# M2219/pyOrbSLAM

Measured on AMD Instinct MI355X. Metric: stereo pairs/s (ORB extract L+R + stereo match), KITTI 1241x376, 1/2/4/8 GPU, higher is better.
Workload: dtype u8; 1 GPU; kitti1241x376_synth_2000f_512pairs; width=1241, height=376, nfeatures=2000, nlevels=8, iniThFAST=20, minThFAST=7, parallelism=512 pairs per GPU on 1 GPU(s) (independent ranks, no data-path collective), handles_per_gpu=4, lanes_per_handle=1

## Files before the change

### pyorbslam_amd/csrc/orbfe_kernels.hip

```cpp
#include <hip/hip_runtime.h>

#include <algorithm>
#include <mutex>
#include <vector>

#include "orbfe_common.h"
#include <type_traits>

#include "orbfe_kernels.h"

namespace orbfe {

constexpr int kBriefSlots = 384;
#define BRIEF_POINT(x, y) x, y,
#define BRIEF_BIT(s0, s1)
constexpr float kBriefSlotXY[2 * kBriefSlots] = {
#include "brief_distinct.inc"
};
#undef BRIEF_POINT
#undef BRIEF_BIT
#define BRIEF_SLOT(s) s,
constexpr int kBriefSlotOrder[kBriefSlots] = {
#include "brief_slot_order.inc"
};
// ... 37 lines not shown
    const uint32_t hi = __builtin_amdgcn_readfirstlane((uint32_t)(a >> 32));
    return __builtin_amdgcn_make_buffer_rsrc((void*)(uintptr_t)(((uint64_t)hi << 32) | lo), 0,
                                             __builtin_amdgcn_readfirstlane(nbytes), 0x00020000);
}

__device__ __forceinline__ __amdgpu_buffer_rsrc_t aligned_rsrc(const void* p, uint32_t nbytes, uint32_t* bias) {
    const uint64_t a = (uint64_t)(uintptr_t)p;
    const uint32_t lo = __builtin_amdgcn_readfirstlane((uint32_t)a);
    const uint32_t hi = __builtin_amdgcn_readfirstlane((uint32_t)(a >> 32));
    *bias = lo & 3u;
    const uint32_t nb = __builtin_amdgcn_readfirstlane(nbytes);
    return __builtin_amdgcn_make_buffer_rsrc((void*)(uintptr_t)(((uint64_t)hi << 32) | (lo & ~3u)), 0, nb + (lo & 3u),
                                             0x00020000);
}

__device__ __forceinline__ void wave_sum2(int& a, int& b) {
    a += __builtin_amdgcn_update_dpp(0, a, 0xB1, 0xF, 0xF, false);
    b += __builtin_amdgcn_update_dpp(0, b, 0xB1, 0xF, 0xF, false);
    a += __builtin_amdgcn_update_dpp(0, a, 0x4E, 0xF, 0xF, false);
    b += __builtin_amdgcn_update_dpp(0, b, 0x4E, 0xF, 0xF, false);
    a += __builtin_amdgcn_update_dpp(0, a, 0x124, 0xF, 0xF, false);
    b += __builtin_amdgcn_update_dpp(0, b, 0x124, 0xF, 0xF, false);
    a += __builtin_amdgcn_update_dpp(0, a, 0x128, 0xF, 0xF, false);
    b += __builtin_amdgcn_update_dpp(0, b, 0x128, 0xF, 0xF, false);
    a = __builtin_amdgcn_readlane(a, 0) + __builtin_amdgcn_readlane(a, 16) + __builtin_amdgcn_readlane(a, 32) +
        __builtin_amdgcn_readlane(a, 48);
    b = __builtin_amdgcn_readlane(b, 0) + __builtin_amdgcn_readlane(b, 16) + __builtin_amdgcn_readlane(b, 32) +
        __builtin_amdgcn_readlane(b, 48);
}

__device__ __forceinline__ int wave_sum(int v) {
    v += __builtin_amdgcn_update_dpp(0, v, 0xB1, 0xF, 0xF, false);
    v += __builtin_amdgcn_update_dpp(0, v, 0x4E, 0xF, 0xF, false);
    v += __builtin_amdgcn_update_dpp(0, v, 0x124, 0xF, 0xF, false);
    v += __builtin_amdgcn_update_dpp(0, v, 0x128, 0xF, 0xF, false);
    return __builtin_amdgcn_readlane(v, 0) + __builtin_amdgcn_readlane(v, 16) + __builtin_amdgcn_readlane(v, 32) +
           __builtin_amdgcn_readlane(v, 48);
}

__device__ __forceinline__ int reflect101(int p, int n) {
    p = p < 0 ? -p : p;
    return p >= n ? 2 * n - 2 - p : p;
}

__device__ __forceinline__ int reflect101_iter(int p, int n) {
    if (n == 1) return 0;
    const int per = 2 * n - 2;
    p = (p < 0 ? -p : p) % per;
    return p >= n ? per - p : p;
}

__device__ __forceinline__ uint32_t resize_tail(uint32_t t, int area) {
    if (!area) return (t + (1u << 21)) >> 22;
    const uint32_t q = t >> 22, r = t & 0x3FFFFFu;
    return q + (r > 0x200000u || (r == 0x200000u && (q & 1u)));
}

__device__ __forceinline__ const uint8_t* level_ptr(const Geo& g, int l, const uint8_t* in, int64_t in_pitch,
                                                    const uint8_t* ws, int img, int* stride) {
    if (l == 0) {
        *stride = g.W;
        return in + (int64_t)img * in_pitch;
    }
    *stride = g.lv[l].pitch;
    return ws + (int64_t)img * g.ws_bytes + g.lv[l].ws_off;
}

__device__ __forceinline__ CellGeo load_cell(const CellGeo* __restrict__ cells, int c) {
    static_assert(sizeof(CellGeo) == 20, "CellGeo layout: 5 dwords");
    const uint32_t* p = (const uint32_t*)(cells + c);
    const uint32_t w0 = p[0], w1 = p[1], w2 = p[2], w3 = p[3], w4 = p[4];
    CellGeo cg;
    cg.level = (int16_t)(w0 & 0xFFFFu);
    cg.kw = (int16_t)(w0 >> 16);
    cg.x0 = (int16_t)(w1 & 0xFFFFu);
    cg.y0 = (int16_t)(w1 >> 16);
    cg.x1 = (int16_t)(w2 & 0xFFFFu);
    cg.y1 = (int16_t)(w2 >> 16);
    cg.slot_off = (int)w3;
    cg.slot_cap = (int)w4;
    return cg;
}

struct KeyDiv {
    uint32_t w, mag, sh;
};
__device__ __forceinline__ KeyDiv key_div(const LevelGeo& L) {
    return KeyDiv{(uint32_t)__builtin_amdgcn_readfirstlane(L.w), (uint32_t)__builtin_amdgcn_readfirstlane((int)L.kmag),
                  (uint32_t)__builtin_amdgcn_readfirstlane(L.ksh)};
}
__device__ __forceinline__ void key_xy(uint32_t k, KeyDiv kd, int& x, int& y) {
    const uint32_t xy = k & 0xFFFFFFu;
    const uint32_t q = __umulhi(xy, kd.mag) >> kd.sh;
    y = (int)q;
    x = (int)(xy - __umul24(q, kd.w));
}

__device__ __forceinline__ void xcd_block(int& bx, int& by) {
    const int nb = gridDim.x * gridDim.y, hw = blockIdx.y * gridDim.x + blockIdx.x, per = nb >> 3;
    const int lb = hw < 8 * per ? (hw & 7) * per + (hw >> 3) : hw;
    by = __builtin_amdgcn_readfirstlane(lb / (int)gridDim.x);
    bx = __builtin_amdgcn_readfirstlane(lb - by * (int)gridDim.x);
}

__device__ int block_excl_scan(int* a, int n, int* tmp) {
    const int t = threadIdx.x;
    const int per = (n + 255) >> 8;
    const int b = t < 256 ? min(t * per, n) : n, e = min(b + per, n);
    int s = 0;
    for (int i = b; i < e; ++i) s += a[i];
    if (t < 256) tmp[t] = s;
    __syncthreads();
    if (t < 64) {
        const int v0 = tmp[4 * t], v1 = tmp[4 * t + 1], v2 = tmp[4 * t + 2], v3 = tmp[4 * t + 3];
        const int tot = v0 + v1 + v2 + v3;
        int inc = tot;
#pragma unroll
        for (int o = 1; o < 64; o <<= 1) {
            const int y = __shfl_up(inc, o, 64);
            if (t >= o) inc += y;
        }
        const int ex = inc - tot;
        tmp[4 * t] = ex;
        tmp[4 * t + 1] = ex + v0;
        tmp[4 * t + 2] = ex + v0 + v1;
        tmp[4 * t + 3] = ex + v0 + v1 + v2;
        if (t == 63) tmp[256] = inc;
    }
    __syncthreads();
    int run = t < 256 ? tmp[t] : 0;
    for (int i = b; i < e; ++i) {
        const int v = a[i];
        a[i] = run;
        run += v;
    }
    const int total = tmp[256];
    __syncthreads();
    return total;
}

__device__ int block_sum(int v, int* red) {
    v = wave_sum(v);
    const int w = threadIdx.x >> 6, nw = blockDim.x >> 6;
    if ((threadIdx.x & 63) == 0) red[w] = v;
    __syncthreads();
    int s = 0;
    for (int i = 0; i < nw; ++i) s += red[i];
    __syncthreads();
    return s;
}

typedef unsigned short us2 __attribute__((ext_vector_type(2)));

__device__ __forceinline__ uint32_t resize_tap3(uint32_t A3, uint32_t aa) {
    typedef __attribute__((address_space(3))) const uint32_t lds_c32;
    const uint32_t o = A3 & 3u;
    lds_c32* w = (lds_c32*)(uintptr_t)(A3 - o);
    const uint32_t x = __builtin_amdgcn_alignbyte(w[1], w[0], o);
    return __builtin_amdgcn_udot2(__builtin_bit_cast(us2, __builtin_amdgcn_perm(x, x, 0x0c010c00u)),
                                  __builtin_bit_cast(us2, aa), 0u, false);
}
constexpr int kRsSlots = 16;

template <bool MULTI>
__global__ __launch_bounds__(512) void k_resize_rows(Geo g, int l, const uint8_t* __restrict__ in, int64_t in_pitch,
                                                     uint8_t* __restrict__ ws, const ResizeX* __restrict__ xt,
                                                     const ResizeY* __restrict__ yt, int wg, int remw, int wgl,
                                                     int* __restrict__ zero_word) {
    extern __shared__ __attribute__((aligned(16))) unsigned char rs_lds[];
    typedef __attribute__((address_space(3))) uint32_t lds_w32;
    typedef __attribute__((address_space(1))) const uint32_t glb_u32;
    lds_w32* s_src = (lds_w32*)(uintptr_t)(__attribute__((address_space(3))) unsigned char*)rs_lds;
    const LevelGeo& L = g.lv[l];
    const LevelGeo& P = g.lv[l - 1];
    int bx, img;
    xcd_block(bx, img);
    const int t = threadIdx.x, nthr = blockDim.x;
    if (zero_word && blockIdx.x == 0 && blockIdx.y == 0 && t == 0) *zero_word = 0;
    const int rows = L.rs_rows;
    const int dy0 = bx * rows, nrow = min(rows, L.h - dy0);
    const int ngrp = (L.w + 3) >> 2;
    int sstride;
    const uint8_t* src = level_ptr(g, l - 1, in, in_pitch, ws, img, &sstride);
    const ResizeY* yb = yt + L.ytab_off + dy0;
    const int ys_lo = yb[0].sy0, ys_hi = yb[nrow - 1].sy1;
    const uintptr_t a0 = (uintptr_t)(src + (int64_t)ys_lo * sstride);
    const int sh0 = (int)(a0 & 3);
    glb_u32* gsrc = (glb_u32*)(a0 - sh0);
    const int ndw = ((ys_hi - ys_lo) * sstride + P.w + sh0 + 3) >> 2;
    typedef __attribute__((address_space(3))) const uint32_t lds_u32;
    const uint32_t src_lds = (uint32_t)(uintptr_t)s_src;
    const int wv = t >> 6, fullw = (nthr >> 6) - remw, nset = fullw / wgl;
    const bool remwave = wv >= fullw;
    const int set = __builtin_amdgcn_readfirstlane(remwave ? 0 : wv / wgl);
    const int rem = ngrp - wg * 64, lane = t & 63;
    const int rstep = remwave ? 64 / rem : nset;
    const int row0 = remwave ? lane / rem : set;
    int ch = remwave ? wg : wv - set * wgl;
    const int ch_step = remwave ? 1 : wgl, ch_end = remwave ? wg + 1 : wg;
    int grp = 0;
    bool own = false;
    uint4 e{}, aa{};
    int sx0 = 0;
    uint32_t d3 = 0;
    auto chunk = [&](int c) {
        grp = remwave ? wg * 64 + lane % rem : c * 64 + lane;
        own = remwave ? lane < rstep * rem : grp < ngrp;
        if (own) {
            const uint4* xg = (const uint4*)(xt + L.xtab_off);
            const uint4 q0 = xg[2 * grp], q1 = xg[2 * grp + 1];
            sx0 = (int)q0.x;
            d3 = q1.z - q0.x;
            auto sel = [&](uint32_t sx) { const uint32_t r = sx - q0.x; return r | ((r + 1) << 16) | 0x0c000c00u; };
            e = uint4{sel(q0.x), sel(q0.z), sel(q1.x), sel(q1.z)};
            aa = uint4{q0.y, q0.w, q1.y, q1.w};
        }
    };
    chunk(ch);
    if (t < 256) {
        const __amdgpu_buffer_rsrc_t rsrc = bounded_rsrc((const void*)(uintptr_t)gsrc, (uint32_t)(4 * ndw));
        for (int base = 0; base < ndw; base += 256 * kRsSlots) {
            const int left = ndw - base;
            uint32_t v[kRsSlots];
#pragma unroll
            for (int k = 0; k < kRsSlots; ++k) {
                v[k] = 0u;
                if (t < left - 256 * k)
                    v[k] = __builtin_amdgcn_raw_buffer_load_b32(rsrc, (uint32_t)(4 * t), (uint32_t)(4 * (base + 256 * k)), 0);
            }
            lds_w32* sp = s_src + base + t;
#pragma unroll
            for (int k = 0; k < kRsSlots; ++k)
                if (t < left - 256 * k) sp[256 * k] = v[k];
        }
    }
    __syncthreads();
    uint8_t* dst = ws + (int64_t)img * g.ws_bytes + L.ws_off + (int64_t)dy0 * L.pitch;
    const __amdgpu_buffer_rsrc_t rd = uniform_rsrc(dst);
    for (;;) {
        if (!own) return;
        const int dx = 4 * grp;
        const bool tail = dx + 3 >= L.xvec;
        const uint32_t lsrc = src_lds + (uint32_t)sh0 + (uint32_t)sx0;
        int psy = -1;
        auto row = [&](int rr, uint32_t (&h0)[4], uint32_t (&h1)[4], bool reuse) {
            const ResizeY y = yb[rr];
            const uint32_t r0 = (uint32_t)((y.sy0 - ys_lo) * sstride), r1 = (uint32_t)((y.sy1 - ys_lo) * sstride);
            const uint32_t B0 = (uint32_t)y.b0 << 12, B1 = (uint32_t)y.b1 << 12;
            auto taps = [&](uint32_t roff, uint32_t (&h)[4]) {
                const uint32_t A = lsrc + roff, o = A & 3u;
                lds_u32* w = (lds_u32*)(uintptr_t)(A - o);
                const uint32_t w0 = w[0], w1 = w[1], w2 = w[2];
                const uint32_t d0 = __builtin_amdgcn_alignbyte(w1, w0, o), d1 = __builtin_amdgcn_alignbyte(w2, w1, o);
                h[0] = __builtin_amdgcn_udot2(__builtin_bit_cast(us2, __builtin_amdgcn_perm(d1, d0, e.x)),
                                              __builtin_bit_cast(us2, aa.x), 0u, false);
                h[1] = __builtin_amdgcn_udot2(__builtin_bit_cast(us2, __builtin_amdgcn_perm(d1, d0, e.y)),
                                              __builtin_bit_cast(us2, aa.y), 0u, false);
                h[2] = __builtin_amdgcn_udot2(__builtin_bit_cast(us2, __builtin_amdgcn_perm(d1, d0, e.z)),
                                              __builtin_bit_cast(us2, aa.z), 0u, false);
                h[3] = L.wide ? resize_tap3(A + d3, aa.w)
                              : __builtin_amdgcn_udot2(__builtin_bit_cast(us2, __builtin_amdgcn_perm(d1, d0, e.w)),
                                                       __builtin_bit_cast(us2, aa.w), 0u, false);
            };
            if (!(reuse && y.sy0 == psy)) taps(r0, h0);
            taps(r1, h1);
            if (reuse) psy = y.sy1;
            uint32_t v[4];
#pragma unroll
            for (int k = 0; k < 4; ++k) v[k] = (__umulhi(h0[k] & ~15u, B0) + __umulhi(h1[k] & ~15u, B1) + 2) >> 2;
            if (tail) {
#pragma unroll
                for (int k = 0; k < 4; ++k)
                    if (dx + k >= L.xvec) v[k] = resize_tail(h0[k] * (B0 >> 12) + h1[k] * (B1 >> 12), L.area);
            }
            __builtin_amdgcn_raw_buffer_store_b32(v[0] | (v[1] << 8) | (v[2] << 16) | (v[3] << 24), rd, (uint32_t)dx,
                                                  (uint32_t)(rr * L.pitch), 0);
        };
        uint32_t ha[4] = {0u, 0u, 0u, 0u}, hb[4] = {0u, 0u, 0u, 0u};
        if (!remwave) {
            const int per = (nrow + nset - 1) / nset, rend = min(set * per + per, nrow);
            psy = -1;
            int rr = set * per;
            for (; rr + 1 < rend; rr += 2) {
                row(rr, ha, hb, true);
                row(rr + 1, hb, ha, true);
            }
            if (rr < rend) row(rr, ha, hb, true);
        } else {
            for (int rr = row0; rr < nrow; rr += rstep) row(rr, ha, hb, false);
        }
        if (!MULTI) return;
        ch += ch_step;
        if (ch >= ch_end) return;
        chunk(ch);
    }
}

constexpr int kCasNT = 1024;
__global__ __launch_bounds__(kCasNT) void k_resize_cascade(Geo g, const uint8_t* __restrict__ in, int64_t in_pitch,
                                                        uint8_t* __restrict__ ws, const ResizeX* __restrict__ xt,
                                                        const ResizeY* __restrict__ yt, const int16_t* __restrict__ tab,
                                                        int offB, int offX, int* __restrict__ zero_word,
                                                        long long* __restrict__ prof) {
    extern __shared__ __attribute__((aligned(16))) unsigned char rs_lds[];
    typedef __attribute__((address_space(3))) const uint32_t lds_u32;
    typedef __attribute__((address_space(3))) uint32_t lds_w32;
    const int strip = blockIdx.x, img = blockIdx.y, t = threadIdx.x, lane = t & 63;
    const int wv = __builtin_amdgcn_readfirstlane(t >> 6), nwv = blockDim.x >> 6;
    if (zero_word && strip == 0 && img == 0 && t == 0) *zero_word = 0;
    long long* pm = prof ? prof + ((int64_t)img * gridDim.x + strip) * 32 : nullptr;
    auto mark = [&](int id) {
        if (pm && t == 0) pm[id] = (long long)wall_clock64();
    };
    mark(0);
    const int L = g.nlevels;
    const int16_t* st = tab + (int64_t)strip * L * 4;
    const uint32_t baseA = (uint32_t)(uintptr_t)(lds_u32*)rs_lds;
    const uint32_t baseB = baseA + (uint32_t)offB;
    typedef unsigned int v4u __attribute__((ext_vector_type(4)));
    typedef __attribute__((address_space(3))) v4u lds_u4;
    typedef __attribute__((address_space(3))) int lds_i32;
    typedef __attribute__((address_space(1))) const v4u glb_u4;
    auto u4 = [](v4u v) { return uint4{v.x, v.y, v.z, v.w}; };
    typedef __attribute__((address_space(1))) const uint32_t glb_u32;
    auto s_xa_of = [&](int par) { return (lds_u4*)(uintptr_t)(baseA + (uint32_t)offX + (uint32_t)(par * 32 * g.rs_ngrp)); };
    auto s_sx_of = [&](int par) {
        return (lds_i32*)(uintptr_t)(baseA + (uint32_t)offX + (uint32_t)(64 * g.rs_ngrp + par * 4 * g.rs_ngrp));
    };
    constexpr int kPre = 1024 / kCasNT;
    uint4 pq0[kPre], pq1[kPre];
    auto prefetch = [&](int l) {
        if (l >= g.nlevels) return;
        glb_u4* xg = (glb_u4*)(xt + g.lv[l].xtab_off);
        const int ng = (g.lv[l].w + 3) >> 2;
#pragma unroll
        for (int k = 0; k < kPre; ++k) {
            const int gi = t + kCasNT * k;
            if (gi < ng) {
                pq0[k] = u4(xg[2 * gi]);
                pq1[k] = u4(xg[2 * gi + 1]);
            }
        }
    };
    auto commit = [&](int l) {
        lds_u4* sxa = s_xa_of(l & 1);
        lds_i32* ssx = s_sx_of(l & 1);
        const int ng = (g.lv[l].w + 3) >> 2;
#pragma unroll
        for (int k = 0; k < kPre; ++k) {
            const int gi = t + kCasNT * k;
            if (gi < ng) {
                const uint4 q0 = pq0[k], q1 = pq1[k];
                auto sel = [&](uint32_t sx) { const uint32_t r = sx - q0.x; return r | ((r + 1) << 16) | 0x0c000c00u; };
                sxa[2 * gi] = v4u{sel(q0.x), sel(q0.z), sel(q1.x), sel(q1.z)};
                sxa[2 * gi + 1] = v4u{q0.y, q0.w, q1.y, q1.w};
                ssx[gi] = (int)(q0.x | ((q1.z - q0.x) << 24));
            }
        }
    };
    prefetch(1);
    uint32_t src_base = baseA, src_sh;
    int src_row0, src_stride;
    {
        const LevelGeo& L1 = g.lv[1];
        const ResizeY* yb = yt + L1.ytab_off;
        const int c0 = st[4], c1 = st[5];
        const int ys_lo = yb[c0].sy0, ys_hi = yb[c1 - 1].sy1;
        const uintptr_t a0 = (uintptr_t)(in + (int64_t)img * in_pitch + (int64_t)ys_lo * g.W);
        src_sh = (uint32_t)(a0 & 3);
        glb_u32* gsrc = (glb_u32*)(a0 - src_sh);
        const int ndw = ((ys_hi - ys_lo) * g.W + g.W + (int)src_sh + 3) >> 2;
        lds_w32* s_src = (lds_w32*)(uintptr_t)baseA;
        for (int base = 0; base < ndw; base += kCasNT * kRsSlots / 2) {
            uint32_t v[kRsSlots / 2];
#pragma unroll
            for (int k = 0; k < kRsSlots / 2; ++k) {
                const int i = base + t + kCasNT * k;
                v[k] = i < ndw ? gsrc[i] : 0u;
            }
#pragma unroll
            for (int k = 0; k < kRsSlots / 2; ++k) {
                const int i = base + t + kCasNT * k;
                if (i < ndw) s_src[i] = v[k];
            }
        }
        src_row0 = ys_lo;
        src_stride = g.W;
    }
    mark(1);
    for (int l = 1; l < L; ++l) {
        const LevelGeo& Lv = g.lv[l];
        const int c0 = st[4 * l], c1 = st[4 * l + 1], o0 = st[4 * l + 2], o1 = st[4 * l + 3];
        const int ngrp = (Lv.w + 3) >> 2, nch = (ngrp + 63) >> 6;
        commit(l);
        prefetch(l + 1);
        const lds_u4* s_xa = s_xa_of(l & 1);
        const lds_i32* s_sx0 = s_sx_of(l & 1);
        const ResizeY* yb = yt + Lv.ytab_off;
        const uint32_t dst_base = (l & 1) ? baseB : baseA;
        __syncthreads();
        mark(2 + l);
        uint8_t* gdst = ws + (int64_t)img * g.ws_bytes + Lv.ws_off;
        const int pitch = Lv.pitch;
        const int lv_wide = __builtin_amdgcn_readfirstlane(Lv.wide), lv_xvec = __builtin_amdgcn_readfirstlane(Lv.xvec),
                  lv_area = __builtin_amdgcn_readfirstlane(Lv.area);
        for (int r = c0 + wv; r < c1; r += nwv) {
            const ResizeY y = yb[r];
            const uint32_t r0 = (uint32_t)((y.sy0 - src_row0) * src_stride), r1 = (uint32_t)((y.sy1 - src_row0) * src_stride);
            const uint32_t B0 = (uint32_t)y.b0 << 12, B1 = (uint32_t)y.b1 << 12;
            const bool own = r >= o0 && r < o1;
            const uint32_t lrow = dst_base + (uint32_t)((r - c0) * pitch);
            uint8_t* grow = gdst + (int64_t)r * pitch;
            for (int ch = 0; ch < nch; ++ch) {
                const int grp = ch * 64 + lane;
                if (grp < ngrp) {
                    const uint4 e = u4(s_xa[2 * grp]), aa = u4(s_xa[2 * grp + 1]);
                    const int sxp = s_sx0[grp];
                    const uint32_t d3 = (uint32_t)sxp >> 24;
                    const uint32_t lsrc = src_base + src_sh + (uint32_t)(sxp & 0xFFFFFF);
                    auto taps = [&](uint32_t roff, uint32_t (&h)[4]) {
                        const uint32_t A = lsrc + roff, o = A & 3u;
                        lds_u32* w = (lds_u32*)(uintptr_t)(A - o);
                        const uint32_t w0 = w[0], w1 = w[1], w2 = w[2];
                        const uint32_t d0 = __builtin_amdgcn_alignbyte(w1, w0, o), d1 = __builtin_amdgcn_alignbyte(w2, w1, o);
                        h[0] = __builtin_amdgcn_udot2(__builtin_bit_cast(us2, __builtin_amdgcn_perm(d1, d0, e.x)),
                                                      __builtin_bit_cast(us2, aa.x), 0u, false);
                        h[1] = __builtin_amdgcn_udot2(__builtin_bit_cast(us2, __builtin_amdgcn_perm(d1, d0, e.y)),
                                                      __builtin_bit_cast(us2, aa.y), 0u, false);
                        h[2] = __builtin_amdgcn_udot2(__builtin_bit_cast(us2, __builtin_amdgcn_perm(d1, d0, e.z)),
                                                      __builtin_bit_cast(us2, aa.z), 0u, false);
                        h[3] = lv_wide ? resize_tap3(A + d3, aa.w)
                                       : __builtin_amdgcn_udot2(__builtin_bit_cast(us2, __builtin_amdgcn_perm(d1, d0, e.w)),
                                                                __builtin_bit_cast(us2, aa.w), 0u, false);
                    };
                    uint32_t h0[4], h1[4];
                    taps(r0, h0);
                    taps(r1, h1);
                    const int dx = 4 * grp;
                    uint32_t v[4];
#pragma unroll
                    for (int k = 0; k < 4; ++k) v[k] = (__umulhi(h0[k] & ~15u, B0) + __umulhi(h1[k] & ~15u, B1) + 2) >> 2;
                    if (dx + 3 >= lv_xvec) {
#pragma unroll
// ... 2725 lines not shown
                if (rtk) mR &= mR - 1;
                else mL &= mL - 1;
                if (slot == k) {
                    own = ownk;
                    rt = rtk;
                    ok = okk;
                }
            }
            const int orow = __shfl(wrow, own, 64), ocl = __shfl(c0l, own, 64), ocr = __shfl(c0r, own, 64);
            const int oct = __shfl(kl.octave, own, 64);
            if (ok && jb < (rt ? 21 : 11)) {
                const int w = s_w[oct], h = s_h[oct], pw = w + 2 * kEdge;
                const int stride = oct == 0 ? g.W : s_pitch[oct];
                int r, c;
                sheared_pos(w, orow, rt ? ocr : ocl, r, c);
                c += jb;
                if (c >= pw) {
                    c -= pw;
                    ++r;
                }
                const uint8_t* base = oct == 0 ? (rt ? lvl0R : lvl0L) : (rt ? wsR : wsL) + s_wsoff[oct];
                const uint16_t e = (uint16_t)(base[(int64_t)reflect101(r - kEdge, h) * stride + reflect101(c - kEdge, w)] + 512u);
                const int gq = (int)(threadIdx.x >> 6) * 4 + (own >> 4), gs = own & 15;
                if (rt) {
                    ((uint16_t*)&sE[gq][gs][0])[jb] = e;
                    if (jb >= 1) ((uint16_t*)&sO[gq][gs][0])[jb - 1] = e;
                } else {
                    ((uint16_t*)&sP[gq][gs][0])[jb] = e;
                }
            }
        }
    }
    __builtin_amdgcn_fence(__ATOMIC_RELEASE, "wavefront");
    __builtin_amdgcn_wave_barrier();
    __builtin_amdgcn_fence(__ATOMIC_ACQUIRE, "wavefront");
    if (do_sad && sl < 11) {
        const int s = sl;
        const int lc = (int)((sP[kq][5][2] >> 16) & 0xFFFFu);
        const uint32_t rw = sE[kq][5][(s + 5) >> 1];
        const int rc = (int)((s & 1) ? (rw & 0xFFFFu) : (rw >> 16));
        const uint32_t d = (uint32_t)(rc - lc) & 0xFFFFu;
        const uint32_t dd = d | (d << 16);
        const int b0 = s >> 1;
        uint32_t acc = 0;
#pragma unroll
        for (int r = 0; r < 11; ++r) {
            const uint32_t* bp = (s & 1) ? &sO[kq][r][b0] : &sE[kq][r][b0];
#pragma unroll
            for (int k = 0; k < 6; ++k) {
                const uint32_t a = __builtin_bit_cast(uint32_t, __builtin_bit_cast(us2, sP[kq][r][k]) +
                                                                    __builtin_bit_cast(us2, dd));
                const uint32_t b = bp[k];
                acc = k < 5 ? __builtin_amdgcn_sad_u16(a, b, acc) : __builtin_amdgcn_sad_u16(a & 0xFFFFu, b & 0xFFFFu, acc);
            }
        }
        sad[kq][s] = (int)acc;
    }
    __builtin_amdgcn_fence(__ATOMIC_RELEASE, "wavefront");
    __builtin_amdgcn_wave_barrier();
    __builtin_amdgcn_fence(__ATOMIC_ACQUIRE, "wavefront");
    if (do_sad && sl == 0) {
        int bi = 0, bd = sad[kq][0];
        for (int s = 1; s < 11; ++s)
            if (sad[kq][s] < bd) {
                bd = sad[kq][s];
                bi = s;
            }
        if (bi != 0 && bi != 10) {
            const int d1 = sad[kq][bi - 1], d2 = sad[kq][bi], d3 = sad[kq][bi + 1];
            const float deltaR = __fdiv_rn((float)(d1 - d3), (float)(2 * (d1 + d3 - 2 * d2)));
            if (!(deltaR < -1.f || deltaR > 1.f)) {
                const float bestuR = __fmul_rn(s_sc[kl.octave], __fadd_rn((float)(scaleduR0 + bi - 5), deltaR));
                const float disparity = __fsub_rn(kl.x, bestuR);
                if (0.f <= disparity && disparity < A.maxD) {
                    if (disparity <= 0.f) {
                        status = 2;
                        uR = (float)((double)kl.x - 0.01);
                        depth = (float)(A.bf / 0.01);
                    } else {
                        status = 1;
                        uR = bestuR;
                        depth = __fdiv_rn(A.bf32, disparity);
                    }
                }
            }
        }
    }
    if (active && sl == 0) {
        const int64_t o = pr * A.out_stride + iL;
        A.u_right[o] = status ? uR : -1.f;
        A.depth[o] = status ? depth : -1.f;
        A.status[o] = (int8_t)status;
        A.match_r[o] = status ? bidx : -1;
    }
}

__global__ __launch_bounds__(256) void k_hamming_matrix(const uint8_t* __restrict__ a, int na, const uint8_t* __restrict__ b,
                                                        int nb, int* __restrict__ out) {
    const int j = blockIdx.x * blockDim.x + threadIdx.x, i = blockIdx.y;
    if (j >= nb) return;
    const uint4* A4 = (const uint4*)(a + (int64_t)i * 32);
    const uint4* B4 = (const uint4*)(b + (int64_t)j * 32);
    const uint4 a0 = A4[0], a1 = A4[1], b0 = B4[0], b1 = B4[1];
    out[(int64_t)i * nb + j] = __popc(a0.x ^ b0.x) + __popc(a0.y ^ b0.y) + __popc(a0.z ^ b0.z) + __popc(a0.w ^ b0.w) +
                               __popc(a1.x ^ b1.x) + __popc(a1.y ^ b1.y) + __popc(a1.z ^ b1.z) + __popc(a1.w ^ b1.w);
}

__global__ __launch_bounds__(256) void k_hamming_search(const uint8_t* __restrict__ q, int nq, const uint8_t* __restrict__ tr,
                                                        const int* __restrict__ off, const int* __restrict__ idx,
                                                        int* __restrict__ best_d, int* __restrict__ best_i,
                                                        int* __restrict__ sec_d, int* __restrict__ sec_i,
                                                        int* __restrict__ all_d) {
    const int qi = blockIdx.x * 4 + (threadIdx.x >> 6), lane = threadIdx.x & 63;
    if (qi >= nq) return;
    const uint4* Q4 = (const uint4*)(q + (int64_t)qi * 32);
    const uint4 a0 = Q4[0], a1 = Q4[1];
    const int b = off[qi], e = off[qi + 1];
    int d1 = 256, p1 = 0x7fffffff, d2 = 256, p2 = 0x7fffffff;
    for (int pos = b + lane; pos < e; pos += 64) {
        const uint4* T4 = (const uint4*)(tr + (int64_t)idx[pos] * 32);
        const uint4 b0 = T4[0], b1 = T4[1];
        const int d = __popc(a0.x ^ b0.x) + __popc(a0.y ^ b0.y) + __popc(a0.z ^ b0.z) + __popc(a0.w ^ b0.w) +
                      __popc(a1.x ^ b1.x) + __popc(a1.y ^ b1.y) + __popc(a1.z ^ b1.z) + __popc(a1.w ^ b1.w);
        if (all_d) all_d[pos] = d;
        if (d < d1) {
            d2 = d1; p2 = p1; d1 = d; p1 = pos;
        } else if (d < d2) {
            d2 = d; p2 = pos;
        }
    }
#pragma unroll
    for (int o = 32; o > 0; o >>= 1) {
        const int od1 = __shfl_xor(d1, o, 64), op1 = __shfl_xor(p1, o, 64);
        const int od2 = __shfl_xor(d2, o, 64), op2 = __shfl_xor(p2, o, 64);
        int cd[4] = {d1, d2, od1, od2}, cp[4] = {p1, p2, op1, op2};
        int bd1 = 257, bp1 = 0x7fffffff, bd2 = 257, bp2 = 0x7fffffff;
#pragma unroll
        for (int k = 0; k < 4; ++k) {
            const bool lt1 = cd[k] < bd1 || (cd[k] == bd1 && cp[k] < bp1);
            const bool lt2 = cd[k] < bd2 || (cd[k] == bd2 && cp[k] < bp2);
            if (lt1) { bd2 = bd1; bp2 = bp1; bd1 = cd[k]; bp1 = cp[k]; }
            else if (lt2) { bd2 = cd[k]; bp2 = cp[k]; }
        }
        d1 = bd1; p1 = bp1; d2 = bd2; p2 = bp2;
    }
    if (lane == 0) {
        best_d[qi] = p1 == 0x7fffffff ? 256 : d1;
        best_i[qi] = p1 == 0x7fffffff ? -1 : idx[p1];
        sec_d[qi] = p2 == 0x7fffffff ? 256 : d2;
        sec_i[qi] = p2 == 0x7fffffff ? -1 : idx[p2];
    }
}

hipError_t launch_resize(const Geo& g, int l, const uint8_t* in, int64_t in_pitch, uint8_t* ws, const ResizeX* xt,
                         const ResizeY* yt, int n_images, hipStream_t s, bool remainder_wave, int* zero_word) {
    const LevelGeo& L = g.lv[l];
    dim3 grid((L.h + L.rs_rows - 1) / L.rs_rows, n_images);
    const int ngrp = (L.w + 3) / 4, rem = ngrp % 64;
    const int wg0 = (ngrp + 63) / 64;
    const int remw = (remainder_wave && ngrp >= 64 && wg0 <= 8 && rem > 0 && rem < 40) ? 1 : 0;
    const int wg = remw ? ngrp / 64 : wg0;
    const int wgl = std::min(wg, 8 - remw);
    const int sets = std::max(1, (4 - remw + wgl - 1) / wgl);
    const int threads = 64 * (wgl * sets + remw);
    if (threads < 256 || threads > 512) return hipErrorInvalidConfiguration;
    auto k = wg > wgl ? k_resize_rows<true> : k_resize_rows<false>;
    hipLaunchKernelGGL(k, grid, dim3(threads), (size_t)L.rs_nsrc * L.rs_sp + 16, s, g, l, in, in_pitch, ws, xt, yt, wg,
                       remw, wgl, zero_word);
    return hipGetLastError();
}

int detect_rp(const Geo& g) { return g.max_rw + 3 <= 48 ? 48 : g.max_rw + 3 <= 64 ? 64 : 96; }

size_t detect_lds_bytes(const Geo& g) {
    return 2 * (size_t)detect_roi_elems(g, detect_rp(g)) + (size_t)detect_rp(g) * (g.max_wh + 2) + 2 * (size_t)g.fd_pq;
}

int detect_cpw(const Geo& g, int n_images) {
    return n_images < kSmallBatchImages || (int64_t)n_images * ((g.ncells + kFdCells - 1) / kFdCells) < 8 * 256
               ? kFdSmallCells
               : kFdCells;
}

template <int RP, int NS>
static void launch_detect_rp(const Geo& g, const CellGeo* cells, const uint8_t* in, int64_t in_pitch, const uint8_t* ws,
                             int* cell_count, uint32_t* slots, int n_images, hipStream_t s, int cpw, int* stats) {
    const dim3 grid((g.ncells + cpw - 1) / cpw, n_images), blk(64);
    const size_t lds = detect_lds_bytes(g);
    auto k = stats ? (cpw == kFdSmallCells ? k_detect<RP, NS, kFdSmallCells, true> : k_detect<RP, NS, kFdCells, true>)
                   : (cpw == kFdSmallCells ? k_detect<RP, NS, kFdSmallCells> : k_detect<RP, NS, kFdCells>);
    hipLaunchKernelGGL(k, grid, blk, lds, s, g, cells, in, in_pitch, ws, cell_count, slots, stats);
}

hipError_t launch_detect(const Geo& g, const CellGeo* cells, const uint8_t* in, int64_t in_pitch, const uint8_t* ws,
                         int* cell_count, uint32_t* slots, int n_images, hipStream_t s, int cells_per_wave, int* stats) {
    const int cpw = cells_per_wave ? cells_per_wave : detect_cpw(g, n_images);
    if (cpw != kFdCells && cpw != kFdSmallCells) return hipErrorInvalidValue;
    const bool tall = g.max_rh > 48;
    switch (detect_rp(g)) {
        case 48:
            if (tall) launch_detect_rp<48, 16>(g, cells, in, in_pitch, ws, cell_count, slots, n_images, s, cpw, stats);
            else launch_detect_rp<48, 12>(g, cells, in, in_pitch, ws, cell_count, slots, n_images, s, cpw, stats);
            break;
        case 64:
            if (tall) launch_detect_rp<64, 16>(g, cells, in, in_pitch, ws, cell_count, slots, n_images, s, cpw, stats);
            else launch_detect_rp<64, 12>(g, cells, in, in_pitch, ws, cell_count, slots, n_images, s, cpw, stats);
            break;
        default: launch_detect_rp<96, 16>(g, cells, in, in_pitch, ws, cell_count, slots, n_images, s, cpw, stats);
    }
    return hipGetLastError();
}

size_t octree_lds_bytes(const Geo& g, int maxcell) {
    const int NC = g.max_ncap;
    int pow2 = 1;
    while (pow2 < NC) pow2 <<= 1;
    return (size_t)8 * NC * 2 + 8 * pow2 + 4 * NC * 2 + 16 * NC + 8 * NC + 4 * NC * 4 + 4 * ((maxcell + 4) & ~3) +
           6 * (size_t)g.oct_keys;
}

size_t octree_bins_lds_bytes(const Geo& g, int maxcell) {
    return ob_carve(g.max_ncap, g.oct_bins_max, maxcell, g.oct_tab_max, g.oct_kblk_max, [](int, size_t) {});
}

constexpr int kMaxDevices = 64;
struct LdsAttr {
    std::vector<std::pair<const void*, int>> raised;
    int get(const void* fn) const {
        for (const auto& e : raised)
            if (e.first == fn) return e.second;
        return 64 * 1024;
    }
    void set(const void* fn, int v) {
        for (auto& e : raised)
            if (e.first == fn) { e.second = v; return; }
        raised.emplace_back(fn, v);
    }
};
static LdsAttr g_lds[kMaxDevices];
static std::mutex g_lds_mu;

static LdsAttr* lds_attr() {
    int dev = 0;
    if (hipGetDevice(&dev) != hipSuccess || dev < 0 || dev >= kMaxDevices) return nullptr;
    return &g_lds[dev];
}

static hipError_t raise_lds(const void* fn, int bytes) {
    std::lock_guard<std::mutex> lk(g_lds_mu);
    LdsAttr* a = lds_attr();
    if (!a) return hipErrorInvalidDevice;
    if (bytes <= a->get(fn)) return hipSuccess;
    if (bytes > 160 * 1024) return hipErrorInvalidValue;
    const hipError_t e = hipFuncSetAttribute(fn, hipFuncAttributeMaxDynamicSharedMemorySize, bytes);
    if (e == hipSuccess) a->set(fn, bytes);
    return e;
}

static int lds_limit(const void* fn) {
    std::lock_guard<std::mutex> lk(g_lds_mu);
    const LdsAttr* a = lds_attr();
    return a ? a->get(fn) : 0;
}

hipError_t prepare_resize_cascade(int lds_bytes) { return raise_lds((const void*)k_resize_cascade, lds_bytes); }

constexpr int kObSmallNT = 512;
static const void* octree_bins_fn(const Geo& g, bool wide) {
    const bool reg = octree_reg_passes(g.max_ncap);
    return wide ? (reg ? (const void*)k_octree_bins<kObSmallNT, true> : (const void*)k_octree_bins<kObSmallNT, false>)
                : (reg ? (const void*)k_octree_bins<kObThreads, true> : (const void*)k_octree_bins<kObThreads, false>);
}

hipError_t prepare_octree(const Geo& g, int maxcell) {
    const size_t nb = octree_bins_lds_bytes(g, maxcell), no = octree_lds_bytes(g, maxcell);
    hipError_t e = hipSuccess;
    if (nb <= 160 * 1024) {
        if ((e = raise_lds(octree_bins_fn(g, false), (int)nb)) != hipSuccess) return e;
        if ((e = raise_lds(octree_bins_fn(g, true), (int)nb)) != hipSuccess) return e;
    }
    if (no <= 160 * 1024) e = raise_lds((const void*)k_octree, (int)no);
    return e;
}

hipError_t launch_resize_cascade(const Geo& g, const uint8_t* in, int64_t in_pitch, uint8_t* ws, const ResizeX* xt,
                                 const ResizeY* yt, const int16_t* strips, int n_strips, int off_b, int off_x,
                                 int lds_bytes, int n_images, hipStream_t s, int* zero_word, long long* prof) {
    if (g.nlevels < 2 || n_images <= 0) return hipSuccess;
    if (lds_bytes > lds_limit((const void*)k_resize_cascade)) return hipErrorInvalidConfiguration;
    hipLaunchKernelGGL(k_resize_cascade, dim3(n_strips, n_images), dim3(kCasNT), (size_t)lds_bytes, s, g, in, in_pitch, ws,
                       xt, yt, strips, off_b, off_x, zero_word, prof);
    return hipGetLastError();
}

hipError_t launch_octree(const Geo& g, const CellGeo* cells, const int* cell_count, const uint32_t* slots,
                         const uint32_t* octab, uint32_t* kd, uint16_t* kn, uint32_t* lvl_kp, int* lvl_count, int* overflow,
                         int maxcell, int n_images, hipStream_t s, int threads, long long* prof) {
    if (g.oct_v == 0) {
        const size_t lds = octree_bins_lds_bytes(g, maxcell);
        if (threads != 0 && threads != kObThreads && threads != kObSmallNT) return hipErrorInvalidValue;
        const bool wide = threads ? threads == kObSmallNT : n_images < kSmallBatchImages;
        const void* fn = octree_bins_fn(g, wide);
        if ((int)lds > lds_limit(fn)) return hipErrorInvalidConfiguration;
        const bool reg = octree_reg_passes(g.max_ncap);
        auto k = wide ? (reg ? k_octree_bins<kObSmallNT, true> : k_octree_bins<kObSmallNT, false>)
                      : (reg ? k_octree_bins<kObThreads, true> : k_octree_bins<kObThreads, false>);
        hipLaunchKernelGGL(k, dim3(n_images, g.nlevels), dim3(wide ? kObSmallNT : kObThreads), lds, s, g, cells, cell_count,
                           slots, octab, lvl_kp, lvl_count, overflow, maxcell, kd, prof);
        return hipGetLastError();
    }
    if (threads != 0) return hipErrorInvalidValue;
    const size_t lds = octree_lds_bytes(g, maxcell);
    if ((int)lds > lds_limit((const void*)k_octree)) return hipErrorInvalidConfiguration;
    hipLaunchKernelGGL(k_octree, dim3(n_images, g.nlevels), dim3(kOctThreads), lds, s, g, cells, cell_count, slots, kd, kn,
                       lvl_kp, lvl_count, overflow, maxcell, prof);
    return hipGetLastError();
}

static int orb_waves(const Geo& g, int kpw) {
// ... 169 lines not shown
```

Baseline: 120,300 pairs/s.

## Specialize resize-rows kernel on thread count, alignment and non-tail fast path

The LDS staging of source rows now uses every thread in the block (compile-time NT) instead of only the first 256. Each staging pass picks a slot count of 8, 16 or 24 based on how much data is left. A compile-time AL4 variant hoists the byte-offset and aligned-address computation out of the per-row taps when the source pitch is a multiple of four. Wavefronts with no tail lanes and no remainder wave take a branch-free path that masks taps once and packs the four output bytes with two adds and a perm. These cut per-row ALU work and staging latency, at the cost of more kernel instantiations and code size.

```diff
diff --git a/pyorbslam_amd/csrc/orbfe_kernels.hip b/pyorbslam_amd/csrc/orbfe_kernels.hip
--- a/pyorbslam_amd/csrc/orbfe_kernels.hip
+++ b/pyorbslam_amd/csrc/orbfe_kernels.hip
@@ -213,17 +213,21 @@
 
 typedef unsigned short us2 __attribute__((ext_vector_type(2)));
 
-__device__ __forceinline__ uint32_t resize_tap3(uint32_t A3, uint32_t aa) {
+__device__ __forceinline__ uint32_t resize_tap3_al(uint32_t W3, uint32_t o, uint32_t aa) {
     typedef __attribute__((address_space(3))) const uint32_t lds_c32;
-    const uint32_t o = A3 & 3u;
-    lds_c32* w = (lds_c32*)(uintptr_t)(A3 - o);
+    lds_c32* w = (lds_c32*)(uintptr_t)W3;
     const uint32_t x = __builtin_amdgcn_alignbyte(w[1], w[0], o);
     return __builtin_amdgcn_udot2(__builtin_bit_cast(us2, __builtin_amdgcn_perm(x, x, 0x0c010c00u)),
                                   __builtin_bit_cast(us2, aa), 0u, false);
 }
+__device__ __forceinline__ uint32_t resize_tap3(uint32_t A3, uint32_t aa) {
+    const uint32_t o = A3 & 3u;
+    return resize_tap3_al(A3 - o, o, aa);
+}
 constexpr int kRsSlots = 16;
-
-template <bool MULTI>
+constexpr int kRsRowSlots = 24;
+
+template <bool MULTI, bool AL4, int NT>
 __global__ __launch_bounds__(512) void k_resize_rows(Geo g, int l, const uint8_t* __restrict__ in, int64_t in_pitch,
                                                      uint8_t* __restrict__ ws, const ResizeX* __restrict__ xt,
                                                      const ResizeY* __restrict__ yt, int wg, int remw, int wgl,
@@ -236,7 +240,7 @@
     const LevelGeo& P = g.lv[l - 1];
     int bx, img;
     xcd_block(bx, img);
-    const int t = threadIdx.x, nthr = blockDim.x;
+    const int t = threadIdx.x;
     if (zero_word && blockIdx.x == 0 && blockIdx.y == 0 && t == 0) *zero_word = 0;
     const int rows = L.rs_rows;
     const int dy0 = bx * rows, nrow = min(rows, L.h - dy0);
@@ -251,7 +255,7 @@
     const int ndw = ((ys_hi - ys_lo) * sstride + P.w + sh0 + 3) >> 2;
     typedef __attribute__((address_space(3))) const uint32_t lds_u32;
     const uint32_t src_lds = (uint32_t)(uintptr_t)s_src;
-    const int wv = t >> 6, fullw = (nthr >> 6) - remw, nset = fullw / wgl;
+    const int wv = t >> 6, fullw = NT / 64 - remw, nset = fullw / wgl;
     const bool remwave = wv >= fullw;
     const int set = __builtin_amdgcn_readfirstlane(remwave ? 0 : wv / wgl);
     const int rem = ngrp - wg * 64, lane = t & 63;
@@ -278,21 +282,30 @@
         }
     };
     chunk(ch);
-    if (t < 256) {
+    {
         const __amdgpu_buffer_rsrc_t rsrc = bounded_rsrc((const void*)(uintptr_t)gsrc, (uint32_t)(4 * ndw));
-        for (int base = 0; base < ndw; base += 256 * kRsSlots) {
+        auto pass = [&](auto nslot, int base, int left) {
+            constexpr int S = decltype(nslot)::value;
+            uint32_t v[S];
+#pragma unroll
+            for (int k = 0; k < S; ++k) {
+                v[k] = 0u;
+                if (t < left - NT * k)
+                    v[k] = __builtin_amdgcn_raw_buffer_load_b32(rsrc, (uint32_t)(4 * t), (uint32_t)(4 * (base + NT * k)), 0);
+            }
+            lds_w32* sp = s_src + base + t;
+#pragma unroll
+            for (int k = 0; k < S; ++k)
+                if (t < left - NT * k) sp[NT * k] = v[k];
+        };
+        for (int base = 0; base < ndw; base += NT * kRsRowSlots) {
             const int left = ndw - base;
-            uint32_t v[kRsSlots];
-#pragma unroll
-            for (int k = 0; k < kRsSlots; ++k) {
-                v[k] = 0u;
-                if (t < left - 256 * k)
-                    v[k] = __builtin_amdgcn_raw_buffer_load_b32(rsrc, (uint32_t)(4 * t), (uint32_t)(4 * (base + 256 * k)), 0);
-            }
-            lds_w32* sp = s_src + base + t;
-#pragma unroll
-            for (int k = 0; k < kRsSlots; ++k)
-                if (t < left - 256 * k) sp[256 * k] = v[k];
+            if (left <= NT * kRsRowSlots / 3)
+                pass(std::integral_constant<int, kRsRowSlots / 3>{}, base, left);
+            else if (left <= NT * (kRsRowSlots * 2 / 3))
+                pass(std::integral_constant<int, kRsRowSlots * 2 / 3>{}, base, left);
+            else
+                pass(std::integral_constant<int, kRsRowSlots>{}, base, left);
         }
     }
     __syncthreads();
@@ -303,53 +316,73 @@
         const int dx = 4 * grp;
         const bool tail = dx + 3 >= L.xvec;
         const uint32_t lsrc = src_lds + (uint32_t)sh0 + (uint32_t)sx0;
-        int psy = -1;
-        auto row = [&](int rr, uint32_t (&h0)[4], uint32_t (&h1)[4], bool reuse) {
-            const ResizeY y = yb[rr];
-            const uint32_t r0 = (uint32_t)((y.sy0 - ys_lo) * sstride), r1 = (uint32_t)((y.sy1 - ys_lo) * sstride);
-            const uint32_t B0 = (uint32_t)y.b0 << 12, B1 = (uint32_t)y.b1 << 12;
-            auto taps = [&](uint32_t roff, uint32_t (&h)[4]) {
-                const uint32_t A = lsrc + roff, o = A & 3u;
-                lds_u32* w = (lds_u32*)(uintptr_t)(A - o);
-                const uint32_t w0 = w[0], w1 = w[1], w2 = w[2];
-                const uint32_t d0 = __builtin_amdgcn_alignbyte(w1, w0, o), d1 = __builtin_amdgcn_alignbyte(w2, w1, o);
-                h[0] = __builtin_amdgcn_udot2(__builtin_bit_cast(us2, __builtin_amdgcn_perm(d1, d0, e.x)),
-                                              __builtin_bit_cast(us2, aa.x), 0u, false);
-                h[1] = __builtin_amdgcn_udot2(__builtin_bit_cast(us2, __builtin_amdgcn_perm(d1, d0, e.y)),
-                                              __builtin_bit_cast(us2, aa.y), 0u, false);
-                h[2] = __builtin_amdgcn_udot2(__builtin_bit_cast(us2, __builtin_amdgcn_perm(d1, d0, e.z)),
-                                              __builtin_bit_cast(us2, aa.z), 0u, false);
-                h[3] = L.wide ? resize_tap3(A + d3, aa.w)
-                              : __builtin_amdgcn_udot2(__builtin_bit_cast(us2, __builtin_amdgcn_perm(d1, d0, e.w)),
-                                                       __builtin_bit_cast(us2, aa.w), 0u, false);
+        const uint32_t lo = lsrc & 3u, lal = lsrc - lo, lo3 = (lsrc + d3) & 3u, lal3 = lsrc + d3 - lo3;
+        auto band = [&](auto tail_c) {
+            constexpr bool TAIL = decltype(tail_c)::value;
+            int psy = -1;
+            auto row = [&](int rr, uint32_t (&h0)[4], uint32_t (&h1)[4], bool reuse) {
+                const ResizeY y = yb[rr];
+                const uint32_t r0 = (uint32_t)((y.sy0 - ys_lo) * sstride), r1 = (uint32_t)((y.sy1 - ys_lo) * sstride);
+                const uint32_t B0 = (uint32_t)y.b0 << 12, B1 = (uint32_t)y.b1 << 12;
+                auto taps = [&](uint32_t roff, uint32_t (&h)[4]) {
+                    const uint32_t A = lsrc + roff, o = AL4 ? lo : A & 3u;
+                    lds_u32* w = (lds_u32*)(uintptr_t)(AL4 ? lal + roff : A - o);
+                    const uint32_t w0 = w[0], w1 = w[1], w2 = w[2];
+                    const uint32_t d0 = __builtin_amdgcn_alignbyte(w1, w0, o), d1 = __builtin_amdgcn_alignbyte(w2, w1, o);
+                    h[0] = __builtin_amdgcn_udot2(__builtin_bit_cast(us2, __builtin_amdgcn_perm(d1, d0, e.x)),
+                                                  __builtin_bit_cast(us2, aa.x), 0u, false);
+                    h[1] = __builtin_amdgcn_udot2(__builtin_bit_cast(us2, __builtin_amdgcn_perm(d1, d0, e.y)),
+                                                  __builtin_bit_cast(us2, aa.y), 0u, false);
+                    h[2] = __builtin_amdgcn_udot2(__builtin_bit_cast(us2, __builtin_amdgcn_perm(d1, d0, e.z)),
+                                                  __builtin_bit_cast(us2, aa.z), 0u, false);
+                    h[3] = L.wide ? (AL4 ? resize_tap3_al(lal3 + roff, lo3, aa.w) : resize_tap3(A + d3, aa.w))
+                                  : __builtin_amdgcn_udot2(__builtin_bit_cast(us2, __builtin_amdgcn_perm(d1, d0, e.w)),
+                                                           __builtin_bit_cast(us2, aa.w), 0u, false);
+                    if (!TAIL) {
+#pragma unroll
+                        for (int k = 0; k < 4; ++k) h[k] &= ~15u;
+                    }
+                };
+                if (!(reuse && y.sy0 == psy)) taps(r0, h0);
+                taps(r1, h1);
+                if (reuse) psy = y.sy1;
+                uint32_t out;
+                if (TAIL) {
+                    uint32_t v[4];
+#pragma unroll
+                    for (int k = 0; k < 4; ++k) v[k] = (__umulhi(h0[k] & ~15u, B0) + __umulhi(h1[k] & ~15u, B1) + 2) >> 2;
+                    if (tail) {
+#pragma unroll
+                        for (int k = 0; k < 4; ++k)
+                            if (dx + k >= L.xvec) v[k] = resize_tail(h0[k] * (B0 >> 12) + h1[k] * (B1 >> 12), L.area);
+                    }
+                    out = v[0] | (v[1] << 8) | (v[2] << 16) | (v[3] << 24);
+                } else {
+                    uint32_t s[4];
+#pragma unroll
+                    for (int k = 0; k < 4; ++k) s[k] = __umulhi(h0[k], B0) + __umulhi(h1[k], B1);
+                    const uint32_t p01 = ((s[1] << 16) + (s[0] + 0x20002u)) >> 2, p23 = ((s[3] << 16) + (s[2] + 0x20002u)) >> 2;
+                    out = __builtin_amdgcn_perm(p23, p01, 0x06040200u);
+                }
+                __builtin_amdgcn_raw_buffer_store_b32(out, rd, (uint32_t)dx, (uint32_t)(rr * L.pitch), 0);
             };
-            if (!(reuse && y.sy0 == psy)) taps(r0, h0);
-            taps(r1, h1);
-            if (reuse) psy = y.sy1;
-            uint32_t v[4];
-#pragma unroll
-            for (int k = 0; k < 4; ++k) v[k] = (__umulhi(h0[k] & ~15u, B0) + __umulhi(h1[k] & ~15u, B1) + 2) >> 2;
-            if (tail) {
-#pragma unroll
-                for (int k = 0; k < 4; ++k)
-                    if (dx + k >= L.xvec) v[k] = resize_tail(h0[k] * (B0 >> 12) + h1[k] * (B1 >> 12), L.area);
-            }
-            __builtin_amdgcn_raw_buffer_store_b32(v[0] | (v[1] << 8) | (v[2] << 16) | (v[3] << 24), rd, (uint32_t)dx,
-                                                  (uint32_t)(rr * L.pitch), 0);
+            uint32_t ha[4] = {0u, 0u, 0u, 0u}, hb[4] = {0u, 0u, 0u, 0u};
+            if (!(TAIL && remwave)) {
+                const int per = (nrow + nset - 1) / nset, rend = min(set * per + per, nrow);
+                int rr = set * per;
+                for (; rr + 1 < rend; rr += 2) {
+                    row(rr, ha, hb, true);
+                    row(rr + 1, hb, ha, true);
+                }
+                if (rr < rend) row(rr, ha, hb, true);
+            } else {
+                for (int rr = row0; rr < nrow; rr += rstep) row(rr, ha, hb, false);
+            }
         };
-        uint32_t ha[4] = {0u, 0u, 0u, 0u}, hb[4] = {0u, 0u, 0u, 0u};
-        if (!remwave) {
-            const int per = (nrow + nset - 1) / nset, rend = min(set * per + per, nrow);
-            psy = -1;
-            int rr = set * per;
-            for (; rr + 1 < rend; rr += 2) {
-                row(rr, ha, hb, true);
-                row(rr + 1, hb, ha, true);
-            }
-            if (rr < rend) row(rr, ha, hb, true);
-        } else {
-            for (int rr = row0; rr < nrow; rr += rstep) row(rr, ha, hb, false);
-        }
+        if (__builtin_amdgcn_ballot_w64(tail || remwave) != 0)
+            band(std::true_type{});
+        else
+            band(std::false_type{});
         if (!MULTI) return;
         ch += ch_step;
         if (ch >= ch_end) return;
@@ -3381,6 +3414,17 @@
     }
 }
 
+template <bool AL4>
+static auto resize_rows_kernel(int threads) {
+    switch (threads) {
+        case 256: return k_resize_rows<false, AL4, 256>;
+        case 320: return k_resize_rows<false, AL4, 320>;
+        case 384: return k_resize_rows<false, AL4, 384>;
+        case 448: return k_resize_rows<false, AL4, 448>;
+        default: return k_resize_rows<false, AL4, 512>;
+    }
+}
+
 hipError_t launch_resize(const Geo& g, int l, const uint8_t* in, int64_t in_pitch, uint8_t* ws, const ResizeX* xt,
                          const ResizeY* yt, int n_images, hipStream_t s, bool remainder_wave, int* zero_word) {
     const LevelGeo& L = g.lv[l];
@@ -3393,7 +3437,9 @@
     const int sets = std::max(1, (4 - remw + wgl - 1) / wgl);
     const int threads = 64 * (wgl * sets + remw);
     if (threads < 256 || threads > 512) return hipErrorInvalidConfiguration;
-    auto k = wg > wgl ? k_resize_rows<true> : k_resize_rows<false>;
+    const bool al4 = (l >= 2 ? g.lv[l - 1].pitch : g.W) % 4 == 0;
+    const auto k = wg > wgl ? (al4 ? k_resize_rows<true, true, 512> : k_resize_rows<true, false, 512>)
+                            : (al4 ? resize_rows_kernel<true>(threads) : resize_rows_kernel<false>(threads));
     hipLaunchKernelGGL(k, grid, dim3(threads), (size_t)L.rs_nsrc * L.rs_sp + 16, s, g, l, in, in_pitch, ws, xt, yt, wg,
                        remw, wgl, zero_word);
     return hipGetLastError();
```

Result: faster. 122,000 pairs/s (median of 6 runs) (+1.4%).
